# fjarri-attic/pyfft

Measured on AMD Instinct MI355X. Metric: batched_c2c_fft_gflops_5NlogN_1d_n2^20, higher is better.
Workload: dtype f32

## Files before the change

### include/mifft.h

```cpp
#ifndef MIFFT_H
#define MIFFT_H

#include <stddef.h>
#include <stdint.h>

#ifdef __cplusplus
extern "C" {
#endif

#define MIFFT_ABI_VERSION 6

#define MIFFT_E_INVALID      (-1)
#define MIFFT_E_UNSUPPORTED  (-2)
#define MIFFT_E_NODEVICE     (-3)

#define MIFFT_F32 0
#define MIFFT_F64 1

#define MIFFT_INTERLEAVED 0
#define MIFFT_SPLIT       1

#define MIFFT_FLAG_SRC_INTERLEAVED 1
#define MIFFT_FLAG_DST_INTERLEAVED 2
#define MIFFT_FLAG_STREAM_SRC 4
// ... 28 lines not shown
    int32_t src;
    int32_t dst;
    int32_t flags;
} mifft_pass;

typedef struct mifft_device_props {
    char    name[256];
    char    gcn_arch[64];
    int32_t compute_units;
    int32_t wavefront_size;
    int32_t max_threads_per_block;
    int32_t max_grid_x;
    int64_t lds_bytes_per_block;
    int64_t total_mem_bytes;
    int32_t clock_khz;
    int32_t l2_bytes;
    int64_t llc_bytes;
    int32_t num_xcc;
    int32_t reserved0;
} mifft_device_props;

int         mifft_abi_version(void);
const char *mifft_last_error(void);
#define MIFFT_DEBUG_NO_ND2 0
#define MIFFT_DEBUG_NO_WAVE 2
#define MIFFT_DEBUG_FORCE_WAVE 3
#define MIFFT_DEBUG_ALT_ROWS 5
#define MIFFT_DEBUG_PAIR 6
#define MIFFT_DEBUG_STORE 7
#define MIFFT_DEBUG_ROWS_ND 8
#define MIFFT_DEBUG_NARROW_TILES 9
#define MIFFT_DEBUG_NO_ROWFIRST 10
#define MIFFT_DEBUG_PAIR_LANES 12
#define MIFFT_DEBUG_KEYS 13
int mifft_debug_set(int32_t key, int32_t value);
int mifft_debug_set_default(int32_t key, int32_t value);
int mifft_debug_get(int32_t key);
int mifft_debug_last_pair_lanes_form(void);

int mifft_device_count(int *count);
int mifft_set_device(int device);
int mifft_get_device(int *device);
int mifft_device_props_get(int device, mifft_device_props *props);
int mifft_malloc(void **ptr, size_t nbytes);
int mifft_free(void *ptr);
int mifft_memset(void *ptr, int value, size_t nbytes, mifft_stream_t stream);
int mifft_memcpy_h2d(void *dst, const void *src, size_t nbytes, mifft_stream_t stream);
int mifft_memcpy_d2h(void *dst, const void *src, size_t nbytes, mifft_stream_t stream);
int mifft_memcpy_d2d(void *dst, const void *src, size_t nbytes, mifft_stream_t stream);
int mifft_host_alloc(void **ptr, size_t nbytes);
int mifft_host_free(void *ptr);
int mifft_memcpy_d2h_async(void *dst, const void *src, size_t nbytes, mifft_stream_t stream);
int mifft_stream_create(mifft_stream_t *stream);
int mifft_stream_destroy(mifft_stream_t stream);
int mifft_stream_sync(mifft_stream_t stream);
int mifft_device_sync(void);
typedef void *mifft_graph_t;
int mifft_stream_is_capturing(mifft_stream_t stream, int32_t *capturing);
int mifft_stream_begin_capture(mifft_stream_t stream);
int mifft_stream_end_capture(mifft_stream_t stream, mifft_graph_t *graph);
int mifft_graph_launch(mifft_graph_t graph, mifft_stream_t stream);
int mifft_graph_destroy(mifft_graph_t graph);
int mifft_event_create(mifft_event_t *event);
int mifft_event_destroy(mifft_event_t event);
int mifft_event_record(mifft_event_t event, mifft_stream_t stream);
int mifft_event_sync(mifft_event_t event);
int mifft_event_query(mifft_event_t event);
int mifft_stream_wait_event(mifft_stream_t stream, mifft_event_t event);
int mifft_event_elapsed_ms(float *ms, mifft_event_t start, mifft_event_t stop);


// ... 163 lines not shown
```

### pyfft_amd/_debug.py

```python
import os


def forced_strategy():
    return os.environ.get("PYFFT_AMD_STRATEGY", "auto")


def pipeline_chunk_bytes(default):
    return (int(os.environ.get("PYFFT_AMD_PIPE_MB", "0")) << 20) or default


def no_nd_generic():
    return bool(os.environ.get("PYFFT_AMD_NO_ND_GENERIC"))


def pipeline_streams(default):
    return int(os.environ.get("PYFFT_AMD_PIPE_STREAMS", "0")) or default


def slab_bytes(default):
    return (int(os.environ.get("PYFFT_AMD_SLAB_MB", "0")) << 20) or default


def no_slabs():
    return bool(os.environ.get("PYFFT_AMD_NO_SLABS"))
# ... 42 lines not shown
    return bool(os.environ.get("PYFFT_AMD_NO_FUSEDP_ALT"))


def no_tiled_kernel():
    return bool(os.environ.get("PYFFT_AMD_NO_TILED"))


def no_mixed_nd():
    return bool(os.environ.get("PYFFT_AMD_NO_MIXED_ND"))


def fused3_lag_ring(lag, ring):
    v = os.environ.get("PYFFT_AMD_FUSED3")
    if v:
        lag, ring = (int(t) for t in v.split(","))
    return lag, ring


def apply_native_switches(native):
    for env, key in (("MIFFT_NO_ND2", native.DEBUG_NO_ND2), ("MIFFT_NO_WAVE", native.DEBUG_NO_WAVE),
                     ("MIFFT_FORCE_WAVE", native.DEBUG_FORCE_WAVE)):
        if os.environ.get(env):
            native.lib.mifft_debug_set_default(key, 1)
    if os.environ.get("MIFFT_STORE"):
        native.lib.mifft_debug_set_default(native.DEBUG_STORE, int(os.environ["MIFFT_STORE"]))
    if os.environ.get("MIFFT_ROWS_ND"):
        native.lib.mifft_debug_set_default(native.DEBUG_ROWS_ND, int(os.environ["MIFFT_ROWS_ND"]))
    if os.environ.get("MIFFT_NARROW_TILES"):
        native.lib.mifft_debug_set_default(native.DEBUG_NARROW_TILES, int(os.environ["MIFFT_NARROW_TILES"]))
    if os.environ.get("MIFFT_PAIR"):
        native.lib.mifft_debug_set_default(native.DEBUG_PAIR, int(os.environ["MIFFT_PAIR"]))
    if os.environ.get("MIFFT_PAIR_LANES"):
        native.lib.mifft_debug_set_default(native.DEBUG_PAIR_LANES, int(os.environ["MIFFT_PAIR_LANES"]))
    if os.environ.get("PYFFT_AMD_NO_SPLIT_ROWFIRST"):
        native.lib.mifft_debug_set_default(native.DEBUG_NO_ROWFIRST, 1)
```

### pyfft_amd/_native.py

```python

import ctypes
import os

_HERE = os.path.dirname(os.path.abspath(__file__))
LIB_PATH = os.path.join(_HERE, "libmifft.so")

ABI_VERSION = 6
MIFFT_MIXED_MAX_STAGES = 12

E_INVALID = -1
E_UNSUPPORTED = -2
E_NODEVICE = -3

F32, F64 = 0, 1
INTERLEAVED, SPLIT = 0, 1
VARIANT_INTERLEAVED_ONLY = 2
VARIANT_SPLIT_ONLY = 3
VARIANT_OUT_OF_PLACE_ONLY = 4
VARIANT_OUT_OF_PLACE_ANY_SIZE = 5
VARIANT_SPLIT_OUT_OF_PLACE = 6
VARIANT_SPLIT_OUT_OF_PLACE_ANY_SIZE = 7
PASS_COL, PASS_ROW, PASS_ND = 0, 1, 2
FLAG_SRC_INTERLEAVED, FLAG_DST_INTERLEAVED = 1, 2
FLAG_STREAM_SRC, FLAG_STREAM_DST = 4, 8
FLAG_WRITE_THROUGH = 32
FLAG_PAIR_WITH_NEXT = 16
HALF_KERNEL_TILE, HALF_KERNEL_ROW, HALF_KERNEL_ND2, HALF_KERNEL_ND = 1, 2, 3, 4
ND_KERNEL_WAVE, ND_KERNEL_ND2Z, ND_KERNEL_ND2, ND_KERNEL_ND2ZP, ND_KERNEL_ND2P, ND_KERNEL_ND2T, ND_KERNEL_ND = 1, 2, 3, 4, 5, 6, 7
FUSED2_COUNTER_STRIDE = 64


def fused2_counter_bytes(outer):
    return FUSED2_COUNTER_STRIDE * 4 * (9 + 2 * int(outer))


DEBUG_NO_ND2, DEBUG_NO_WAVE, DEBUG_FORCE_WAVE, DEBUG_ALT_ROWS, DEBUG_PAIR, DEBUG_STORE = 0, 2, 3, 5, 6, 7
DEBUG_ROWS_ND = 8
DEBUG_NARROW_TILES = 9
DEBUG_NO_ROWFIRST = 10
DEBUG_PAIR_LANES = 12
DEBUG_KEYS = 13


class MifftPass(ctypes.Structure):
    _fields_ = [
        ("kind", ctypes.c_int32),
        ("precision", ctypes.c_int32),
        ("layout", ctypes.c_int32),
        ("inverse", ctypes.c_int32),
        ("L", ctypes.c_int32),
        ("variant", ctypes.c_int32),
        ("M", ctypes.c_int64),
        ("S", ctypes.c_int64),
        ("outer", ctypes.c_int64),
        ("outer_stride_in", ctypes.c_int64),
        ("outer_stride_out", ctypes.c_int64),
        ("scale", ctypes.c_double),
        ("tw_L", ctypes.c_void_p),
        ("tw_lo", ctypes.c_void_p),
        ("tw_hi", ctypes.c_void_p),
        ("tw_shift", ctypes.c_int32),
        ("src", ctypes.c_int32),
        ("dst", ctypes.c_int32),
        ("flags", ctypes.c_int32),
    ]


class MifftCopy(ctypes.Structure):
    _fields_ = [
        ("precision", ctypes.c_int32),
        ("ndim", ctypes.c_int32),
        ("dims", ctypes.c_int64 * 6),
        ("src_stride", ctypes.c_int64 * 6),
        ("dst_stride", ctypes.c_int64 * 6),
# ... 63 lines not shown
class MifftRealPost(ctypes.Structure):
    _fields_ = [
        ("precision", ctypes.c_int32),
        ("inverse", ctypes.c_int32),
        ("nx", ctypes.c_int32),
        ("ny", ctypes.c_int32),
        ("nz", ctypes.c_int32),
        ("reserved", ctypes.c_int32),
        ("outer", ctypes.c_int64),
        ("stride_in", ctypes.c_int64),
        ("stride_out", ctypes.c_int64),
        ("in_", ctypes.c_void_p),
        ("out", ctypes.c_void_p),
        ("tw", ctypes.c_void_p),
        ("scale", ctypes.c_double),
    ]


_vp = ctypes.c_void_p
_vpp = ctypes.POINTER(ctypes.c_void_p)
_i32 = ctypes.c_int32
_sz = ctypes.c_size_t
_pass_p = ctypes.POINTER(MifftPass)
_sync_p = ctypes.POINTER(MifftFusedSync)
_buf3 = ctypes.c_void_p * 3

PROTOTYPES = {
    "mifft_abi_version": (ctypes.c_int, []),
    "mifft_last_error": (ctypes.c_char_p, []),
    "mifft_debug_set": (ctypes.c_int, [_i32, _i32]),
    "mifft_debug_set_default": (ctypes.c_int, [_i32, _i32]),
    "mifft_debug_get": (ctypes.c_int, [_i32]),
    "mifft_debug_last_pair_lanes_form": (ctypes.c_int, []),
    "mifft_device_count": (ctypes.c_int, [ctypes.POINTER(ctypes.c_int)]),
    "mifft_set_device": (ctypes.c_int, [ctypes.c_int]),
    "mifft_get_device": (ctypes.c_int, [ctypes.POINTER(ctypes.c_int)]),
    "mifft_device_props_get": (ctypes.c_int, [ctypes.c_int, ctypes.POINTER(MifftDeviceProps)]),
    "mifft_malloc": (ctypes.c_int, [_vpp, _sz]),
    "mifft_free": (ctypes.c_int, [_vp]),
    "mifft_memset": (ctypes.c_int, [_vp, ctypes.c_int, _sz, _vp]),
    "mifft_memcpy_h2d": (ctypes.c_int, [_vp, _vp, _sz, _vp]),
    "mifft_memcpy_d2h": (ctypes.c_int, [_vp, _vp, _sz, _vp]),
    "mifft_memcpy_d2d": (ctypes.c_int, [_vp, _vp, _sz, _vp]),
    "mifft_host_alloc": (ctypes.c_int, [_vpp, _sz]),
    "mifft_host_free": (ctypes.c_int, [_vp]),
    "mifft_memcpy_d2h_async": (ctypes.c_int, [_vp, _vp, _sz, _vp]),
    "mifft_stream_create": (ctypes.c_int, [_vpp]),
    "mifft_stream_destroy": (ctypes.c_int, [_vp]),
    "mifft_stream_sync": (ctypes.c_int, [_vp]),
    "mifft_device_sync": (ctypes.c_int, []),
    "mifft_stream_is_capturing": (ctypes.c_int, [_vp, ctypes.POINTER(ctypes.c_int32)]),
    "mifft_stream_begin_capture": (ctypes.c_int, [_vp]),
    "mifft_stream_end_capture": (ctypes.c_int, [_vp, _vpp]),
    "mifft_graph_launch": (ctypes.c_int, [_vp, _vp]),
    "mifft_graph_destroy": (ctypes.c_int, [_vp]),
    "mifft_event_create": (ctypes.c_int, [_vpp]),
    "mifft_event_destroy": (ctypes.c_int, [_vp]),
    "mifft_event_record": (ctypes.c_int, [_vp, _vp]),
    "mifft_event_sync": (ctypes.c_int, [_vp]),
    "mifft_event_query": (ctypes.c_int, [_vp]),
    "mifft_stream_wait_event": (ctypes.c_int, [_vp, _vp]),
    "mifft_event_elapsed_ms": (ctypes.c_int, [ctypes.POINTER(ctypes.c_float), _vp, _vp]),
    "mifft_nd_max_points_for": (ctypes.c_int, [_i32]),
    "mifft_nd_shape_supported": (ctypes.c_int, [_i32, _i32, _i32, _i32, _i32]),
    "mifft_pass_supported": (ctypes.c_int, [_i32, _i32, _i32, _i32]),
    "mifft_launch_pass": (ctypes.c_int, [_pass_p, _vp, _vp, _vp, _vp, _vp]),
# ... 94 lines not shown
```

### pyfft_amd/csrc/fft_col2.hpp

```cpp
#pragma once
#include "fft_tile.hpp"

namespace mifft {

template <int A, int E, typename T> __device__ __forceinline__ cplx<T> mul_w16A(cplx<T> v) {
    if constexpr (A == 4)
        return mul_w64<E, T>(v);
    else
        return mul_w32<E, T>(v);
}

template <typename T> struct ColStageTw {
    cplx<T> s1, s2, s3, s4, s5, s6, s7, s8;
    __device__ __forceinline__ void init(const cplx<T>* twL, int i0, int step = 1) {
        load(twL, i0, step);
        finish();
    }
    __device__ __forceinline__ void load(const cplx<T>* twL, int i0, int step = 1) {
        s1 = twL[step * i0]; s2 = twL[2 * step * i0]; s4 = twL[4 * step * i0]; s8 = twL[8 * step * i0];
    }
    __device__ __forceinline__ void finish() {
        s3 = cmul<T>(s1, s2); s5 = cmul<T>(s4, s1); s6 = cmul<T>(s4, s2); s7 = cmul<T>(s4, s3);
    }
    template <int k> __device__ __forceinline__ cplx<T> get() const {
        if constexpr (k == 1) return s1;
        else if constexpr (k == 2) return s2;
        else if constexpr (k == 3) return s3;
        else if constexpr (k == 4) return s4;
        else if constexpr (k == 5) return s5;
        else if constexpr (k == 6) return s6;
        else if constexpr (k == 7) return s7;
        else if constexpr (k == 8) return s8;
        else if constexpr (k == 9) return cmul<T>(s8, s1);
        else if constexpr (k == 10) return cmul<T>(s8, s2);
        else if constexpr (k == 11) return cmul<T>(s8, s3);
        else if constexpr (k == 12) return cmul<T>(s8, s4);
        else if constexpr (k == 13) return cmul<T>(s8, s5);
        else if constexpr (k == 14) return cmul<T>(s8, s6);
        else return cmul<T>(s8, s7);
    }
};

template <int A, bool TR, int ESZ = 8> struct Col2Lds {
    static constexpr int PITCH = TR ? 17 : 16;
    static constexpr int BUF = 16 * 16 * PITCH;
    static constexpr bool DOUBLE = A > 2 && ESZ <= 8;
    static constexpr bool HALF = ESZ > 8;
    static constexpr int ELEMS = HALF ? (BUF + 1) / 2 : (DOUBLE ? 2 : 1) * BUF;
};

struct TileNoHook {
    __device__ __forceinline__ void operator()() const {}
};

__device__ __forceinline__ void pair_swap(cplx<float>& lo, cplx<float>& hi) {
    const float lx = lo.x, ly = lo.y, hx = hi.x, hy = hi.y;
    const auto rx = __builtin_amdgcn_permlane32_swap(__builtin_bit_cast(unsigned, lx), __builtin_bit_cast(unsigned, hx), false, false);
    const auto ry = __builtin_amdgcn_permlane32_swap(__builtin_bit_cast(unsigned, ly), __builtin_bit_cast(unsigned, hy), false, false);
    const unsigned ax = rx[0], bx = rx[1], ay = ry[0], by = ry[1];
    lo.x = __builtin_bit_cast(float, ax); hi.x = __builtin_bit_cast(float, bx);
    lo.y = __builtin_bit_cast(float, ay); hi.y = __builtin_bit_cast(float, by);
}

template <typename T, int A, bool TR, bool TW, bool SPLIT, bool WT = false, bool NTIN = false, bool NTOUT = false,
          bool SPLIT_OUT = SPLIT, bool WIDE = false, bool PAIR_IN = false, bool PAIR_OUT = false, typename LdsPtr = cplx<T>*,
          typename Hook = TileNoHook>
__device__ __forceinline__ void col2_tile(const TileArgs& a, const long long o_in, const long long o_out,
                                          const long long rem0, LdsPtr lds, Hook hook = Hook(), const int tid_in = -1) {
    constexpr int L = A * 256;
    constexpr int PPT = A * 16;
    constexpr int PITCH = Col2Lds<A, TR, sizeof(cplx<T>)>::PITCH;
    constexpr int BUF = Col2Lds<A, TR, sizeof(cplx<T>)>::BUF;
    constexpr bool kDoubleBuf = Col2Lds<A, TR, sizeof(cplx<T>)>::DOUBLE;
    constexpr bool kHalf = Col2Lds<A, TR, sizeof(cplx<T>)>::HALF;
    static_assert(!(PAIR_IN || PAIR_OUT) || (sizeof(T) == 4 && !WIDE && !kHalf), "paired lanes: fp32 16-column tiles only");
    static_assert(!PAIR_IN || !SPLIT, "PAIR_IN: interleaved input only");
    static_assert(!PAIR_OUT || !SPLIT_OUT, "PAIR_OUT: interleaved output only");
    typedef T vec4 __attribute__((ext_vector_type(4)));

    int tid = tid_in >= 0 ? tid_in : (int)threadIdx.x;
    asm volatile("" : "+v"(tid));
    const int upper = (tid >> 5) & 1;
    const int pair_i = ((tid & 7) << 1) | upper, pair_j = ((tid >> 6) << 2) | ((tid >> 3) & 3);
    const int cg = PAIR_IN ? pair_i : WIDE ? (tid & 31) : (tid & 15), b0 = PAIR_IN ? pair_j : WIDE ? (tid >> 5) : (tid >> 4);
    const int c = cg & 15;
    if constexpr (WIDE) lds = lds + (cg >> 4) * Col2Lds<A, TR, sizeof(cplx<T>)>::ELEMS;
    int logMS = a.logMS, logS = a.logS;
    asm volatile("" : "+s"(logMS), "+s"(logS));
    const cplx<T>* twL = reinterpret_cast<const cplx<T>*>(a.tw_L);
    const T csign = a.inverse ? (T)-1 : (T)1;

    cplx<T> v[PPT];
    {
        const long long ubase = o_in * a.ostride_in + rem0;
        const unsigned voff = (((unsigned)b0 << logMS) + (unsigned)cg);
        if constexpr (PAIR_IN) {
            const char* src = reinterpret_cast<const char*>(reinterpret_cast<const cplx<T>*>(a.in0) + ubase);
            const unsigned vb = ((((unsigned)b0 + (upper ? 16u * A : 0u)) << logMS) + (unsigned)(cg & ~1)) * (unsigned)sizeof(cplx<T>);
            static_for<PPT / 2>([&](auto mm) {
                constexpr int k = 2 * mm, ia = k >> 4, b1 = k & 15;
                const char* p = src + (((long long)(b1 * 16 * A + ia * 16) << logMS) * (long long)sizeof(cplx<T>));
                vec4 w;
                if constexpr (NTIN)
                    w = __builtin_nontemporal_load(reinterpret_cast<const vec4*>(p + vb));
                else
                    w = *reinterpret_cast<const vec4*>(p + vb);
                v[k].x = w.x; v[k].y = w.y; v[k + 1].x = w.z; v[k + 1].y = w.w;
            });
        } else if constexpr (!SPLIT) {
            const char* src = reinterpret_cast<const char*>(reinterpret_cast<const cplx<T>*>(a.in0) + ubase);
            const unsigned vb = voff * (unsigned)sizeof(cplx<T>);
            static_for<PPT>([&](auto kk) {
                constexpr int k = kk, ia = k >> 4, b1 = k & 15;
                const char* p = src + (((long long)(b1 * 16 * A + ia * 16) << logMS) * (long long)sizeof(cplx<T>));
                if constexpr (NTIN)
                    v[k] = __builtin_nontemporal_load(reinterpret_cast<const cplx<T>*>(p + vb));
                else
                    v[k] = *reinterpret_cast<const cplx<T>*>(p + vb);
            });
        } else {
            const char* sre = reinterpret_cast<const char*>(reinterpret_cast<const T*>(a.in0) + ubase);
            const char* sim = reinterpret_cast<const char*>(reinterpret_cast<const T*>(a.in1) + ubase);
            const unsigned vb = voff * (unsigned)sizeof(T);
            static_for<PPT>([&](auto kk) {
                constexpr int k = kk, ia = k >> 4, b1 = k & 15;
                const long long off = ((long long)(b1 * 16 * A + ia * 16) << logMS) * (long long)sizeof(T);
                if constexpr (NTIN) {
                    v[k].x = __builtin_nontemporal_load(reinterpret_cast<const T*>(sre + off + vb));
                    v[k].y = __builtin_nontemporal_load(reinterpret_cast<const T*>(sim + off + vb));
                } else {
                    v[k].x = *reinterpret_cast<const T*>(sre + off + vb);
                    v[k].y = *reinterpret_cast<const T*>(sim + off + vb);
                }
            });
// ... 56 lines not shown
                constexpr int ia = aa;
                t[ia] = v[ia * 16 + qb1];
            });
            Dft<A, T>::run(t);
            v[qb1] = t[0];
            static_for<A - 1>([&](auto qq) {
                constexpr int qa = qq + 1;
                v[qa * 16 + qb1] = cmul<T>(t[qa], twA[qq]);
            });
        });
    }
    __builtin_amdgcn_sched_barrier(0);
    hook();

    const int u = PAIR_OUT ? (TR ? pair_i : pair_j) : TR ? c : b0;
    const int c2 = PAIR_OUT ? (TR ? pair_j : pair_i) : TR ? b0 : c;
    const int c2g = WIDE ? ((cg & 16) + c2) : c2;
    const int c2s = (PAIR_OUT && !TR) ? (c2g & ~1) : c2g;
    const int us = (PAIR_OUT && TR) ? (u & ~1) : u;
    const long long l0 = rem0 >> logS;
    const long long jp0 = rem0 & ((1ll << logS) - 1);
    const unsigned dl = (unsigned)(((rem0 + c2s) >> logS) - l0);
    const unsigned djp = (unsigned)(((rem0 + c2s) & ((1ll << logS) - 1)) - jp0);
    const unsigned l = PAIR_OUT ? (unsigned)((rem0 + c2g) >> logS) : (unsigned)l0 + dl;
    const T sx = (T)a.scale;
    const T sy = a.inverse ? -sx : sx;
    cplx<T> sxy;
    sxy.x = sx;
    sxy.y = sy;
    const cplx<T>* twlo = reinterpret_cast<const cplx<T>*>(a.tw_lo);
    const cplx<T>* twhi = reinterpret_cast<const cplx<T>*>(a.tw_hi);
    const int tw_shift = a.tw_shift;
    const unsigned lomask = (1u << tw_shift) - 1u;
    const long long oubase = TR ? (a.ostride_out * o_out + rem0 * L) : (a.ostride_out * o_out + ((l0 * L) << logS) + jp0);
    const unsigned ovoff = (TR ? ((unsigned)c2g * L + (unsigned)us) : ((((unsigned)dl * L + (unsigned)us) << logS) + djp)) +
                           ((PAIR_OUT && upper) ? (TR ? 16u * A : ((16u * A) << logS)) : 0u);

    cplx<T> nlo[TW ? 4 : 1], nhi[TW ? 4 : 1], sstep_lo, sstep_hi;
    auto look_ahead = [&](auto qq) {
        constexpr int qa = qq;
        if constexpr (TW) {
            static_for<4>([&](auto jj) {
                constexpr int j = jj;
                const unsigned e = l * (unsigned)(qa * 16 + u + 64 * A * j);
                nlo[j] = twlo[e & lomask];
                nhi[j] = twhi[e >> tw_shift];
            });
        }
    };
    if constexpr (TW) {
        const unsigned e = l * (16u * A);
        sstep_lo = twlo[e & lomask];
        sstep_hi = twhi[e >> tw_shift];
        look_ahead(IC<0>{});
        __builtin_amdgcn_sched_barrier(0);
    }

    static_for<A>([&](auto rr) {
        constexpr int qa = rr;
        LdsPtr buf = lds + (kDoubleBuf ? (qa & 1) * BUF : 0);
        if constexpr (!kDoubleBuf && qa > 0) __syncthreads();
        cplx<T> x[16];
        if constexpr (!kHalf) {
            static_for<16>([&](auto ss) {
                constexpr int qb1 = ss;
                if constexpr (TR)
                    buf[(b0 * 16 + c) * PITCH + qb1] = v[qa * 16 + qb1];
                else
                    buf[(b0 * 16 + qb1) * 16 + c] = v[qa * 16 + qb1];
// ... 27 lines not shown
                        w = sb[(bi * 16 + c2) * PITCH + u];
                    else
                        w = sb[(bi * 16 + u) * 16 + c2];
                    if constexpr (comp == 0) x[bi].x = w; else x[bi].y = w;
                });
            });
        }
        cplx<T> anchor[TW ? 4 : 1];
        cplx<T> sstep;
        if constexpr (TW) {
            static_for<4>([&](auto jj) { anchor[jj] = cmul<T>(nlo[jj], nhi[jj]); });
            sstep = cmul<T>(sstep_lo, sstep_hi);
            __builtin_amdgcn_sched_barrier(0);
            if constexpr (qa + 1 < A) {
                look_ahead(IC<qa + 1>{});
                __builtin_amdgcn_sched_barrier(0);
            }
        }
        Dft<16, T>::run(x);
        if constexpr (TW) {
            static_for<4>([&](auto jj) {
                constexpr int j = jj;
                cplx<T> cur = anchor[j];
                static_for<4>([&](auto ii) {
                    constexpr int qb0 = 4 * j + ii;
                    x[qb0] = cmul<T>(x[qb0], cur);
                    if constexpr (ii < 3) cur = cmul<T>(cur, sstep);
                });
            });
        }
        if constexpr (PAIR_OUT) {
            static_for<8>([&](auto hh) {
                constexpr int qb0 = 2 * hh;
                const long long gu = TR ? (oubase + qb0 * 16 * A + 16 * qa)
                                        : (oubase + ((long long)(qb0 * 16 * A + 16 * qa) << logS));
                cplx<T> r0 = x[qb0] * sxy, r1 = x[qb0 + 1] * sxy;
                pair_swap(r0, r1);
                vec4 w;
                w.x = r0.x; w.y = r0.y; w.z = r1.x; w.w = r1.y;
                char* p = reinterpret_cast<char*>(reinterpret_cast<cplx<T>*>(a.out0) + gu);
                if constexpr (WT)
                    store_b128_sc1(p, ovoff * (unsigned)sizeof(cplx<T>), __builtin_bit_cast(unsigned __attribute__((ext_vector_type(4))), w));
                else if constexpr (NTOUT)
                    __builtin_nontemporal_store(w, reinterpret_cast<vec4*>(p + ovoff * (unsigned)sizeof(cplx<T>)));
                else
                    *reinterpret_cast<vec4*>(p + ovoff * (unsigned)sizeof(cplx<T>)) = w;
            });
        } else {
        static_for<16>([&](auto qq) {
            constexpr int qb0 = qq;
            const long long gu = TR ? (oubase + qb0 * 16 * A + 16 * qa)
                                    : (oubase + ((long long)(qb0 * 16 * A + 16 * qa) << logS));
            const cplx<T> r = x[qb0] * sxy;
            if constexpr (!SPLIT_OUT) {
                char* p = reinterpret_cast<char*>(reinterpret_cast<cplx<T>*>(a.out0) + gu);
                if constexpr (WT) {
                    if constexpr (sizeof(cplx<T>) == 8)
                        __hip_atomic_store(reinterpret_cast<unsigned long long*>(p + ovoff * (unsigned)sizeof(cplx<T>)),
                                           __builtin_bit_cast(unsigned long long, r), __ATOMIC_RELAXED, __HIP_MEMORY_SCOPE_AGENT);
                    else
                        store_wt<T>(p, ovoff * (unsigned)sizeof(cplx<T>), r);
                } else if constexpr (NTOUT) {
                    __builtin_nontemporal_store(r, reinterpret_cast<cplx<T>*>(p + ovoff * (unsigned)sizeof(cplx<T>)));
                } else {
                    *reinterpret_cast<cplx<T>*>(p + ovoff * (unsigned)sizeof(cplx<T>)) = r;
                }
            } else {
                char* pr = reinterpret_cast<char*>(reinterpret_cast<T*>(a.out0) + gu);
// ... 53 lines not shown
```

### pyfft_amd/csrc/fft_fused2.hpp

```cpp
#pragma once
#include "fft_col2.hpp"
#include "fft_col2w.hpp"
#include "fft_col3.hpp"

namespace mifft {

constexpr unsigned kFusedCS = 64u;

struct FusedCtl {
    unsigned* counters;
    unsigned* counters_next;
    unsigned* err;
    unsigned lines;
    unsigned batch;
    unsigned lag;
    unsigned ring;
    unsigned tiles0;
    unsigned tiles1;
};

struct FusedArgs {
    TileArgs p0;
    TileArgs p1;
    FusedCtl c;
// ... 146 lines not shown
        if (it.pass == 2u) {
            fused_flush(pend);
            continue;
        }
        if (it.pass == 0u) {
            if (it.dep != nullptr) fused_wait_ge<false>(it.dep, it.target, seen, err, pend);
            else fused_flush(pend);
            if constexpr (EARLY) tile0(it.t, it.slot, it.tile, hook);
            else tile0(it.t, it.slot, it.tile, TileNoHook());
            pend.ctr = wdone + kFusedCS * it.t;
        } else {
            fused_wait_ge<true>(it.dep, it.target, seen, err, pend);
            if constexpr (EARLY) tile1(it.slot, it.t, it.tile, hook);
            else tile1(it.slot, it.t, it.tile, TileNoHook());
            fused_signal_read(rdone + kFusedCS * it.t);
        }
    }
    fused_flush(pend);
}

template <unsigned PER0, unsigned PER1, bool EARLY, typename TILE0, typename TILE1>
__device__ __forceinline__ void fused_loop(const FusedCtl& f, unsigned* s_item, TILE0&& tile0, TILE1&& tile1) {
    if (f.counters_next != nullptr) {
        for (unsigned i = blockIdx.x * blockDim.x + threadIdx.x; i < f.lines; i += gridDim.x * blockDim.x) {
            f.counters_next[i * kFusedCS] = 0u;
            f.counters_next[i * kFusedCS + 1u] = 0u;
        }
    }
    FusedPending pend = {};
    fused_list<PER0, PER1, EARLY>(f, s_item, tile0, tile1, pend);
}

constexpr int kPairIn = 1, kPairOut = 2;
template <typename T, int A0, int A1, bool SPLIT, int NT, int PAIR0 = 0, int PAIR1 = 0>
__global__ void __launch_bounds__(256, 2) fft_fused2_kernel(const FusedArgs f) {
    static_assert((PAIR0 | PAIR1) == 0 || (sizeof(T) == 4 && A0 == 4 && A1 == 4 && !SPLIT && NT == 1), "paired lanes: <float, 4, 4, false, 1> only");
    constexpr int E0 = Col2Lds<A0, true, sizeof(cplx<T>)>::ELEMS, E1 = Col2Lds<A1, false, sizeof(cplx<T>)>::ELEMS;
    __shared__ __attribute__((aligned(16))) cplx<T> lds[E0 > E1 ? E0 : E1];
    __shared__ unsigned s_item;
    constexpr unsigned per0 = A0 > A1 ? 1u : (unsigned)(A1 / A0);
    constexpr unsigned per1 = A1 > A0 ? 1u : (unsigned)(A0 / A1);
    fused_loop<per0, per1, !SPLIT && sizeof(T) == 4>(
        f.c, &s_item,
        [&](unsigned t, unsigned slot, unsigned tile, auto hook) {
            col2_tile<T, A0, true, true, SPLIT, true, NT != 0, false, false, false, (PAIR0 & kPairIn) != 0, (PAIR0 & kPairOut) != 0>(
                f.p0, (long long)t, (long long)slot, (long long)tile * 16, lds, hook);
        },
        [&](unsigned slot, unsigned t, unsigned tile, auto hook) {
            col2_tile<T, A1, false, false, false, NT == 2, false, NT == 1, SPLIT, false, (PAIR1 & kPairIn) != 0, (PAIR1 & kPairOut) != 0>(
                f.p1, (long long)slot, (long long)t, (long long)tile * 16, lds, hook);
        });
}

template <int A0, int A1, bool TWOD, bool NT = false, bool SPLIT = true>
__global__ void __launch_bounds__(512, 2) fft_fused2s_kernel(const FusedArgs f) {
    constexpr int E0 = Col2Lds<A0, true, sizeof(cplx<float>)>::ELEMS, E1 = Col2Lds<A1, TWOD, sizeof(cplx<float>)>::ELEMS;
    constexpr int E = E0 > E1 ? E0 : E1;
    __shared__ __attribute__((aligned(16))) cplx<float> lds[2 * E];
    __shared__ unsigned s_item;
    constexpr unsigned per0 = A0 > A1 ? 1u : (unsigned)(A1 / A0);
    constexpr unsigned per1 = A1 > A0 ? 1u : (unsigned)(A0 / A1);
    fused_loop<per0, per1, false>(
        f.c, &s_item,
        [&](unsigned t, unsigned slot, unsigned item, auto hook) {
            int tid = threadIdx.x;
            asm volatile("" : "+v"(tid));
            col2_tile<float, A0, true, !TWOD, SPLIT, true, NT, false, false, true>(f.p0, (long long)t, (long long)slot, (long long)item * 32, lds, hook, tid);
        },
        [&](unsigned slot, unsigned t, unsigned item, auto hook) {
            int tid = threadIdx.x;
            asm volatile("" : "+v"(tid));
            col2_tile<float, A1, TWOD, false, false, false, false, NT, SPLIT, true>(f.p1, (long long)slot, (long long)t, (long long)item * 32, lds, hook, tid);
        });
}

template <int A0, int A1>
__global__ void __launch_bounds__(256, 2) fft_fused2w_kernel(const FusedArgs f) {
    constexpr int E0 = Col2wLds<true>::ELEMS, E1 = Col2wLds<false>::ELEMS;
    __shared__ __attribute__((aligned(16))) cplx<float> lds[E0 > E1 ? E0 : E1];
    __shared__ unsigned s_item;
    constexpr unsigned per0 = A0 > A1 ? 1u : (unsigned)(A1 / A0);
    constexpr unsigned per1 = A1 > A0 ? 1u : (unsigned)(A0 / A1);
// ... 97 lines not shown
```

### pyfft_amd/csrc/fft_fused2_f32.hip

```cpp
#include "../../include/mifft.h"
#include "mifft_internal.h"
#include "fft_fused2.hpp"

namespace {
constexpr int kPairLanesDefault = 3;
int launch_1024(const mifft::FusedArgs* f, unsigned grid, hipStream_t s) {
    constexpr int kPairAll = mifft::kPairIn | mifft::kPairOut;
    const int sw = mifft_debug_get(MIFFT_DEBUG_PAIR_LANES);
    int form = sw == 0 ? kPairLanesDefault : sw - 1;
    if (form != 0 && form != 3) return -2;
    if ((((uintptr_t)f->p0.in0 | (uintptr_t)f->p1.out0) & 15) != 0) form = 0;
    if (form == 3) hipLaunchKernelGGL((mifft::fft_fused2_kernel<float, 4, 4, false, 1, kPairAll, kPairAll>), dim3(grid), dim3(256), 0, s, *f);
    else hipLaunchKernelGGL((mifft::fft_fused2_kernel<float, 4, 4, false, 1>), dim3(grid), dim3(256), 0, s, *f);
    mifft_note_pair_lanes_form(form);
    return (int)hipGetLastError();
}

template <int A0, int A1> int launch(const mifft::FusedArgs* f, int split, unsigned grid, hipStream_t s) {
    if constexpr (A0 < A1) {
        return -2;
    } else {
        const int store = mifft_debug_get(MIFFT_DEBUG_STORE);
        if (mifft_debug_get(MIFFT_DEBUG_NARROW_TILES) == 1 || store == 2 || store == 3) return -2;
        if (split) {
            hipLaunchKernelGGL((mifft::fft_fused2s_kernel<A0, A1, false, true>), dim3(grid), dim3(512), 0, s, *f);
        } else if constexpr (A0 == 4 && A1 == 4) {
            return launch_1024(f, grid, s);
        } else if constexpr (A0 == 4) {
            hipLaunchKernelGGL((mifft::fft_fused2_kernel<float, A0, A1, false, 1>), dim3(grid), dim3(256), 0, s, *f);
        } else {
            return -2;
        }
        return (int)hipGetLastError();
    }
}
}

extern "C" int mifft_fused2_f32_launch(int L0, int L1, const mifft::FusedArgs* f, int split, unsigned grid, hipStream_t s) {
    if (L0 == 2048 && L1 == 2048) {
        if (split) hipLaunchKernelGGL((mifft::fft_fused3_kernel<float, 4, 4, true, true>), dim3(grid), dim3(512), 0, s, *f);
        else hipLaunchKernelGGL((mifft::fft_fused3_kernel<float, 4, 4, false, true>), dim3(grid), dim3(512), 0, s, *f);
        return (int)hipGetLastError();
    }
    if (L0 == 2048 && L1 == 1024) {
        if (split) hipLaunchKernelGGL((mifft::fft_fused3_kernel<float, 4, 2, true, true>), dim3(grid), dim3(512), 0, s, *f);
        else hipLaunchKernelGGL((mifft::fft_fused3_kernel<float, 4, 2, false, true>), dim3(grid), dim3(512), 0, s, *f);
        return (int)hipGetLastError();
// ... 27 lines not shown
```

### pyfft_amd/csrc/mifft_internal.h

```cpp
#pragma once
#include <hip/hip_runtime.h>
#include "../../include/mifft.h"
#include "fft_tile.hpp"
#include "fft_fused2.hpp"
#include "fft_nd.hpp"
#include "fft_wave.hpp"
#include "fft_pair.hpp"
#include "fft_nd2t.hpp"
#include "fft_fusedp.hpp"

extern "C" {
int mifft_dispatch_col_f32(int L, int tr, int variant, const mifft::TileArgs* a, hipStream_t s, int query_only);
int mifft_dispatch_row_f32(int L, int variant, const mifft::TileArgs* a, hipStream_t s, int query_only);
int mifft_dispatch_col_f64(int L, int tr, int variant, const mifft::TileArgs* a, hipStream_t s, int query_only);
int mifft_dispatch_row_f64(int L, int variant, const mifft::TileArgs* a, hipStream_t s, int query_only);
int mifft_nd_max_points(int f64);
int mifft_nd_launch(int f64, long long n, const mifft::NdArgs* a, hipStream_t s);
int mifft_nd2_f32_supported(int x, int y, int z);
int mifft_nd2_f32_launch(int x, int y, int z, const mifft::TileArgs* a, hipStream_t s);
int mifft_nd2_f64_supported(int x, int y, int z);
int mifft_nd2_f64_launch(int x, int y, int z, const mifft::TileArgs* a, hipStream_t s);
int mifft_fused2_f32_launch(int L0, int L1, const mifft::FusedArgs* f, int split, unsigned grid, hipStream_t s);
void mifft_note_pair_lanes_form(int form);
int mifft_fused2dw_f32(int ny, int nx, const mifft::FusedArgs* f, unsigned grid, hipStream_t s, int query, unsigned* tiles0, unsigned* tiles1);
int mifft_fused2r_f32(int ny, int nx, const mifft::FusedArgs* f, unsigned grid, hipStream_t s, int query);
int mifft_fused2w_f32_launch(int L0, int L1, const mifft::FusedArgs* f, unsigned grid, hipStream_t s);
int mifft_fused2d_f32_launch(int ny, int nx, const mifft::FusedArgs* f, int split, unsigned grid, hipStream_t s);
int mifft_fused3d_f64_launch(int ny, int nx, const mifft::FusedArgs* f, int split, unsigned grid, hipStream_t s);
int mifft_fusedx_f64(int L0, int L1, const mifft::FusedArgs* f, unsigned grid, hipStream_t s, int query, unsigned* tiles0, unsigned* tiles1);
int mifft_fused3_f64_launch(int L0, int L1, const mifft::FusedArgs* f, int split, unsigned grid, hipStream_t s);
int mifft_aux_copy_launch(const struct mifft_copy* c, const void* s0, const void* s1, void* d0, void* d1, hipStream_t s);
int mifft_aux_mul_rows_launch(int f64, void* a, const void* b, long long rows, long long n, hipStream_t s);
int mifft_aux_mul_spectrum_launch(int f64, void* data, const void* spectrum, long long items, long long points, long long spectrum_pitch,
                                  int correlate, double scale, hipStream_t s);
int mifft_aux_mismatch_launch(const void* a, const void* b, unsigned long long words, unsigned long long* count, hipStream_t s);
int mifft_aux_zero_launch(void* p, unsigned long long nbytes, hipStream_t s);
int mifft_wave_supported(int f64, int N);
int mifft_wave_launch(int f64, int N, const mifft::WaveArgs* a, int max_blocks, hipStream_t s);
int mifft_wave_16x16_launch(const mifft::WaveArgs* a, int max_blocks, hipStream_t s);
int mifft_pair_f64(int kind, int k0, int k1, int k2, int split, const mifft::PairArgs* a, hipStream_t s, int query, int* width);
int mifft_pair_f32(int kind, int k0, int k1, int k2, int split, const mifft::PairArgs* a, hipStream_t s, int query, int* width);
int mifft_fusedp(int f64, int split, int x, int y, int z, const mifft::FusedPairArgs* f, unsigned grid, hipStream_t s, int query, int* r0,
                 unsigned* tiles0, unsigned* tiles1);
int mifft_fusedp_more(int f64, int split, int x, int y, int z, const mifft::FusedPairArgs* f, unsigned grid, hipStream_t s, int query, int* r0,
                      unsigned* tiles0, unsigned* tiles1);
int mifft_nd2t(int f64, int x, int y, int z, const mifft::TileArgs* a, const mifft::TiledGeom* g, hipStream_t s, int query);
int mifft_nd2t_split_in(int f64, int x, int y, int z, const mifft::TileArgs* a, const mifft::TiledGeom* g, hipStream_t s, int query);
int mifft_nd2t_split(int f64, int x, int y, int z, const mifft::TileArgs* a, const mifft::TiledGeom* g, hipStream_t s, int query);
int mifft_nd2p(int f64, int x, int y, int z, const mifft::TileArgs* a, hipStream_t s, int query);
int mifft_nd2zp(int f64, int x, int y, int z, const mifft::TileArgs* a, hipStream_t s, int query);
int mifft_mixed_supported_impl(int f64, int n);
int mifft_mixed_radices_impl(int n, int32_t* radix);
int mifft_mixed_launch(int f64, int n, long long rows, long long stride_in, long long stride_out, long long inner, const void* in,
                       void* out, const void* tw, int flags, double scale, hipStream_t s);
int mifft_mixed_long_split_impl(int f64, long long n, int* n1, int* n2);
int mifft_mixed_long_launch(int f64, int n1, int n2, long long batch, const void* in, void* mid, void* out, const void* tw1, const void* tw2,
// ... 52 lines not shown
```

### pyfft_amd/csrc/mifft_runtime.cpp

```cpp
#include <hip/hip_runtime.h>
#include <hsa/hsa.h>
#include <hsa/hsa_ext_amd.h>

#include <atomic>
#include <cstdarg>
#include <cstdio>
#include <cstring>
#include <cstdlib>
#include <initializer_list>

#include "../../include/mifft.h"
#include "mifft_internal.h"
#include "fft_conv_row.hpp"

namespace {

thread_local char g_err[512] = "";
std::atomic<int> g_debug_default[MIFFT_DEBUG_KEYS];
thread_local int t_debug_value[MIFFT_DEBUG_KEYS];
thread_local unsigned t_debug_mask = 0;
thread_local int t_pair_lanes_form = -1;
struct DebugSwitches {
    int operator[](int key) const {
        return ((t_debug_mask >> key) & 1u) ? t_debug_value[key] : g_debug_default[key].load(std::memory_order_relaxed);
    }
};
const DebugSwitches g_debug;

int set_err(int code, const char* fmt, ...) {
    va_list ap;
    va_start(ap, fmt);
    vsnprintf(g_err, sizeof(g_err), fmt, ap);
    va_end(ap);
    return code;
}

int hip_check(hipError_t e, const char* what) {
    if (e == hipSuccess) return 0;
    return set_err((int)e, "%s: %s (%d)", what, hipGetErrorString(e), (int)e);
}

int launched(int rc) {
    if (rc == -1) return set_err(MIFFT_E_INVALID, "grid too large");
    return hip_check((hipError_t)rc, "kernel launch");
}

bool is_pow2(long long v) { return v > 0 && (v & (v - 1)) == 0; }
bool bad_precision(int precision) { return precision != MIFFT_F32 && precision != MIFFT_F64; }
long long complex_bytes(int precision) { return precision == MIFFT_F64 ? 16 : 8; }
bool misaligned(uintptr_t mask, std::initializer_list<const void*> ptrs) {
    uintptr_t all = 0;
    for (const void* p : ptrs) all |= (uintptr_t)p;
    return (all & mask) != 0;
}
// ... 382 lines not shown
    c->tiles1 = tiles1;
    if (!sync->counters_next) {
        hipStreamCaptureStatus st = hipStreamCaptureStatusNone;
        if (hipStreamIsCapturing(stream, &st) == hipSuccess && st == hipStreamCaptureStatusActive) {
            const int rz = mifft_aux_zero_launch(sync->counters, MIFFT_FUSED2_COUNTER_BYTES(outer), stream);
            return hip_check((hipError_t)rz, "kernel launch");
        }
        return hip_check(hipMemsetAsync(sync->counters, 0, MIFFT_FUSED2_COUNTER_BYTES(outer), stream), "hipMemsetAsync");
    }
    return 0;
}

template <typename F> F* row_dispatcher(int32_t precision, F* f32, F* f64) { return precision == MIFFT_F64 ? f64 : f32; }

}

extern "C" {

int mifft_abi_version(void) { return MIFFT_ABI_VERSION; }
int mifft_debug_set(int32_t key, int32_t value) {
    if (!debug_key_ok(key)) return set_err(MIFFT_E_INVALID, "bad debug key %d", key);
    t_debug_value[key] = value;
    t_debug_mask |= 1u << key;
    return 0;
}
int mifft_debug_set_default(int32_t key, int32_t value) {
    if (!debug_key_ok(key)) return set_err(MIFFT_E_INVALID, "bad debug key %d", key);
    g_debug_default[key].store(value, std::memory_order_relaxed);
    return 0;
}
int mifft_debug_get(int32_t key) { return (key >= 0 && key < MIFFT_DEBUG_KEYS) ? g_debug[key] : 0; }
void mifft_note_pair_lanes_form(int form) { t_pair_lanes_form = form; }
int mifft_debug_last_pair_lanes_form(void) { return t_pair_lanes_form; }
const char* mifft_last_error(void) { return g_err; }

int mifft_device_count(int* count) {
    if (!count) return set_err(MIFFT_E_INVALID, "null argument");
    hipError_t e = hipGetDeviceCount(count);
    if (e == hipErrorNoDevice) {
        *count = 0;
        (void)hipGetLastError();
        return 0;
    }
    return hip_check(e, "hipGetDeviceCount");
}
int mifft_set_device(int device) { return hip_check(hipSetDevice(device), "hipSetDevice"); }
int mifft_get_device(int* device) { return hip_check(hipGetDevice(device), "hipGetDevice"); }

int mifft_device_props_get(int device, mifft_device_props* props) {
    if (!props) return set_err(MIFFT_E_INVALID, "null argument");
    hipDeviceProp_t p;
    int rc = hip_check(hipGetDeviceProperties(&p, device), "hipGetDeviceProperties");
    if (rc) return rc;
    memset(props, 0, sizeof(*props));
    snprintf(props->name, sizeof(props->name), "%s", p.name);
    snprintf(props->gcn_arch, sizeof(props->gcn_arch), "%s", p.gcnArchName);
    props->compute_units = p.multiProcessorCount;
    props->wavefront_size = p.warpSize;
    props->max_threads_per_block = p.maxThreadsPerBlock;
    props->max_grid_x = p.maxGridSize[0];
    props->lds_bytes_per_block = (int64_t)p.sharedMemPerBlock;
    props->total_mem_bytes = (int64_t)p.totalGlobalMem;
    props->clock_khz = p.clockRate;
    props->l2_bytes = p.l2CacheSize;
    probe_memory_system(p, &props->llc_bytes, &props->num_xcc);
    return 0;
// ... 961 lines not shown
```

Baseline: 22600.

## Add bit-permuted ring layout for fused 1024x1024 intermediate buffer

Adds a compile-time bit-permutation layout for the intermediate ring buffer between the two stages of the fused persistent 1024x1024 fp32 kernel. The intermediate is stored as [i][j][n2%16][k1%16], so each 16x16 tile written by stage one and read by stage two is contiguous rather than strided by 1024. The goal is better write/read locality, fewer DRAM pages and fewer cache lines touched per tile. The layout is on by default for the paired-lane form, with a debug switch to fall back, and it adds index arithmetic plus a risk of addressing mistakes in the permuted offsets.

```diff
diff --git a/include/mifft.h b/include/mifft.h
--- a/include/mifft.h
+++ b/include/mifft.h
@@ -84,11 +84,13 @@
 #define MIFFT_DEBUG_NARROW_TILES 9
 #define MIFFT_DEBUG_NO_ROWFIRST 10
 #define MIFFT_DEBUG_PAIR_LANES 12
-#define MIFFT_DEBUG_KEYS 13
+#define MIFFT_DEBUG_RING_LAYOUT 13
+#define MIFFT_DEBUG_KEYS 14
 int mifft_debug_set(int32_t key, int32_t value);
 int mifft_debug_set_default(int32_t key, int32_t value);
 int mifft_debug_get(int32_t key);
 int mifft_debug_last_pair_lanes_form(void);
+int mifft_debug_last_ring_layout(void);
 
 int mifft_device_count(int *count);
 int mifft_set_device(int device);
diff --git a/pyfft_amd/_debug.py b/pyfft_amd/_debug.py
--- a/pyfft_amd/_debug.py
+++ b/pyfft_amd/_debug.py
@@ -98,5 +98,7 @@
         native.lib.mifft_debug_set_default(native.DEBUG_PAIR, int(os.environ["MIFFT_PAIR"]))
     if os.environ.get("MIFFT_PAIR_LANES"):
         native.lib.mifft_debug_set_default(native.DEBUG_PAIR_LANES, int(os.environ["MIFFT_PAIR_LANES"]))
+    if os.environ.get("MIFFT_RING_LAYOUT"):
+        native.lib.mifft_debug_set_default(native.DEBUG_RING_LAYOUT, int(os.environ["MIFFT_RING_LAYOUT"]))
     if os.environ.get("PYFFT_AMD_NO_SPLIT_ROWFIRST"):
         native.lib.mifft_debug_set_default(native.DEBUG_NO_ROWFIRST, 1)
diff --git a/pyfft_amd/_native.py b/pyfft_amd/_native.py
--- a/pyfft_amd/_native.py
+++ b/pyfft_amd/_native.py
@@ -39,7 +39,8 @@
 DEBUG_NARROW_TILES = 9
 DEBUG_NO_ROWFIRST = 10
 DEBUG_PAIR_LANES = 12
-DEBUG_KEYS = 13
+DEBUG_RING_LAYOUT = 13
+DEBUG_KEYS = 14
 
 
 class MifftPass(ctypes.Structure):
@@ -169,6 +170,7 @@
     "mifft_debug_set_default": (ctypes.c_int, [_i32, _i32]),
     "mifft_debug_get": (ctypes.c_int, [_i32]),
     "mifft_debug_last_pair_lanes_form": (ctypes.c_int, []),
+    "mifft_debug_last_ring_layout": (ctypes.c_int, []),
     "mifft_device_count": (ctypes.c_int, [ctypes.POINTER(ctypes.c_int)]),
     "mifft_set_device": (ctypes.c_int, [ctypes.c_int]),
     "mifft_get_device": (ctypes.c_int, [ctypes.POINTER(ctypes.c_int)]),
diff --git a/pyfft_amd/csrc/fft_col2.hpp b/pyfft_amd/csrc/fft_col2.hpp
--- a/pyfft_amd/csrc/fft_col2.hpp
+++ b/pyfft_amd/csrc/fft_col2.hpp
@@ -1,5 +1,6 @@
 #pragma once
 #include "fft_tile.hpp"
+#include "fft_ring_layout.hpp"
 
 namespace mifft {
 
@@ -63,8 +64,8 @@
 }
 
 template <typename T, int A, bool TR, bool TW, bool SPLIT, bool WT = false, bool NTIN = false, bool NTOUT = false,
-          bool SPLIT_OUT = SPLIT, bool WIDE = false, bool PAIR_IN = false, bool PAIR_OUT = false, typename LdsPtr = cplx<T>*,
-          typename Hook = TileNoHook>
+          bool SPLIT_OUT = SPLIT, bool WIDE = false, bool PAIR_IN = false, bool PAIR_OUT = false, int RING = 0,
+          typename LdsPtr = cplx<T>*, typename Hook = TileNoHook>
 __device__ __forceinline__ void col2_tile(const TileArgs& a, const long long o_in, const long long o_out,
                                           const long long rem0, LdsPtr lds, Hook hook = Hook(), const int tid_in = -1) {
     constexpr int L = A * 256;
@@ -76,6 +77,10 @@
     static_assert(!(PAIR_IN || PAIR_OUT) || (sizeof(T) == 4 && !WIDE && !kHalf), "paired lanes: fp32 16-column tiles only");
     static_assert(!PAIR_IN || !SPLIT, "PAIR_IN: interleaved input only");
     static_assert(!PAIR_OUT || !SPLIT_OUT, "PAIR_OUT: interleaved output only");
+    constexpr bool kRingOut = RING != 0 && TR, kRingIn = RING != 0 && !TR;
+    static_assert(RING >= 0 && RING < kRingLayouts, "no such ring layout");
+    static_assert(RING == 0 || (sizeof(T) == 4 && A == 4 && !SPLIT && !SPLIT_OUT && PAIR_IN && PAIR_OUT && (TR ? (TW && WT) : (!TW && !WT))),
+                  "ring layouts: the paired-lane fp32 1024 x 1024 persistent kernel only");
     typedef T vec4 __attribute__((ext_vector_type(4)));
 
     int tid = tid_in >= 0 ? tid_in : (int)threadIdx.x;
@@ -95,11 +100,14 @@
         const long long ubase = o_in * a.ostride_in + rem0;
         const unsigned voff = (((unsigned)b0 << logMS) + (unsigned)cg);
         if constexpr (PAIR_IN) {
-            const char* src = reinterpret_cast<const char*>(reinterpret_cast<const cplx<T>*>(a.in0) + ubase);
-            const unsigned vb = ((((unsigned)b0 + (upper ? 16u * A : 0u)) << logMS) + (unsigned)(cg & ~1)) * (unsigned)sizeof(cplx<T>);
+            const char* src = reinterpret_cast<const char*>(reinterpret_cast<const cplx<T>*>(a.in0) +
+                                                            (kRingIn ? o_in * a.ostride_in + (long long)ring_offset<RING>(0u, (unsigned)rem0) : ubase));
+            const unsigned vb = (kRingIn ? ring_offset<RING>(((unsigned)b0 & 15u) + (upper ? 16u * A : 0u), (unsigned)(cg & 14))
+                                         : ((((unsigned)b0 + (upper ? 16u * A : 0u)) << logMS) + (unsigned)(cg & ~1))) * (unsigned)sizeof(cplx<T>);
             static_for<PPT / 2>([&](auto mm) {
                 constexpr int k = 2 * mm, ia = k >> 4, b1 = k & 15;
-                const char* p = src + (((long long)(b1 * 16 * A + ia * 16) << logMS) * (long long)sizeof(cplx<T>));
+                const char* p = src + (kRingIn ? (long long)ring_offset<RING>(b1 * 16 * A + ia * 16, 0u) * (long long)sizeof(cplx<T>)
+                                               : (((long long)(b1 * 16 * A + ia * 16) << logMS) * (long long)sizeof(cplx<T>)));
                 vec4 w;
                 if constexpr (NTIN)
                     w = __builtin_nontemporal_load(reinterpret_cast<const vec4*>(p + vb));
@@ -222,9 +230,12 @@
     const cplx<T>* twhi = reinterpret_cast<const cplx<T>*>(a.tw_hi);
     const int tw_shift = a.tw_shift;
     const unsigned lomask = (1u << tw_shift) - 1u;
-    const long long oubase = TR ? (a.ostride_out * o_out + rem0 * L) : (a.ostride_out * o_out + ((l0 * L) << logS) + jp0);
-    const unsigned ovoff = (TR ? ((unsigned)c2g * L + (unsigned)us) : ((((unsigned)dl * L + (unsigned)us) << logS) + djp)) +
-                           ((PAIR_OUT && upper) ? (TR ? 16u * A : ((16u * A) << logS)) : 0u);
+    const long long oubase = kRingOut ? (a.ostride_out * o_out + (long long)ring_offset<RING>((unsigned)rem0, 0u))
+                             : TR     ? (a.ostride_out * o_out + rem0 * L)
+                                      : (a.ostride_out * o_out + ((l0 * L) << logS) + jp0);
+    const unsigned ovoff = kRingOut ? ring_offset<RING>((unsigned)c2g & 15u, ((unsigned)us & 14u) + (upper ? 16u * A : 0u))
+                                    : (TR ? ((unsigned)c2g * L + (unsigned)us) : ((((unsigned)dl * L + (unsigned)us) << logS) + djp)) +
+                                          ((PAIR_OUT && upper) ? (TR ? 16u * A : ((16u * A) << logS)) : 0u);
 
     cplx<T> nlo[TW ? 4 : 1], nhi[TW ? 4 : 1], sstep_lo, sstep_hi;
     auto look_ahead = [&](auto qq) {
@@ -318,8 +329,9 @@
         if constexpr (PAIR_OUT) {
             static_for<8>([&](auto hh) {
                 constexpr int qb0 = 2 * hh;
-                const long long gu = TR ? (oubase + qb0 * 16 * A + 16 * qa)
-                                        : (oubase + ((long long)(qb0 * 16 * A + 16 * qa) << logS));
+                const long long gu = kRingOut ? (oubase + (long long)ring_offset<RING>(0u, qb0 * 16 * A + 16 * qa))
+                                     : TR     ? (oubase + qb0 * 16 * A + 16 * qa)
+                                              : (oubase + ((long long)(qb0 * 16 * A + 16 * qa) << logS));
                 cplx<T> r0 = x[qb0] * sxy, r1 = x[qb0 + 1] * sxy;
                 pair_swap(r0, r1);
                 vec4 w;
diff --git a/pyfft_amd/csrc/fft_fused2.hpp b/pyfft_amd/csrc/fft_fused2.hpp
--- a/pyfft_amd/csrc/fft_fused2.hpp
+++ b/pyfft_amd/csrc/fft_fused2.hpp
@@ -202,9 +202,10 @@
 }
 
 constexpr int kPairIn = 1, kPairOut = 2;
-template <typename T, int A0, int A1, bool SPLIT, int NT, int PAIR0 = 0, int PAIR1 = 0>
+template <typename T, int A0, int A1, bool SPLIT, int NT, int PAIR0 = 0, int PAIR1 = 0, int RING = 0>
 __global__ void __launch_bounds__(256, 2) fft_fused2_kernel(const FusedArgs f) {
     static_assert((PAIR0 | PAIR1) == 0 || (sizeof(T) == 4 && A0 == 4 && A1 == 4 && !SPLIT && NT == 1), "paired lanes: <float, 4, 4, false, 1> only");
+    static_assert(RING == 0 || (PAIR0 == (kPairIn | kPairOut) && PAIR1 == (kPairIn | kPairOut)), "ring layouts: <float, 4, 4, false, 1> with every stream paired only");
     constexpr int E0 = Col2Lds<A0, true, sizeof(cplx<T>)>::ELEMS, E1 = Col2Lds<A1, false, sizeof(cplx<T>)>::ELEMS;
     __shared__ __attribute__((aligned(16))) cplx<T> lds[E0 > E1 ? E0 : E1];
     __shared__ unsigned s_item;
@@ -213,11 +214,11 @@
     fused_loop<per0, per1, !SPLIT && sizeof(T) == 4>(
         f.c, &s_item,
         [&](unsigned t, unsigned slot, unsigned tile, auto hook) {
-            col2_tile<T, A0, true, true, SPLIT, true, NT != 0, false, false, false, (PAIR0 & kPairIn) != 0, (PAIR0 & kPairOut) != 0>(
+            col2_tile<T, A0, true, true, SPLIT, true, NT != 0, false, false, false, (PAIR0 & kPairIn) != 0, (PAIR0 & kPairOut) != 0, RING>(
                 f.p0, (long long)t, (long long)slot, (long long)tile * 16, lds, hook);
         },
         [&](unsigned slot, unsigned t, unsigned tile, auto hook) {
-            col2_tile<T, A1, false, false, false, NT == 2, false, NT == 1, SPLIT, false, (PAIR1 & kPairIn) != 0, (PAIR1 & kPairOut) != 0>(
+            col2_tile<T, A1, false, false, false, NT == 2, false, NT == 1, SPLIT, false, (PAIR1 & kPairIn) != 0, (PAIR1 & kPairOut) != 0, RING>(
                 f.p1, (long long)slot, (long long)t, (long long)tile * 16, lds, hook);
         });
 }
diff --git a/pyfft_amd/csrc/fft_fused2_f32.hip b/pyfft_amd/csrc/fft_fused2_f32.hip
--- a/pyfft_amd/csrc/fft_fused2_f32.hip
+++ b/pyfft_amd/csrc/fft_fused2_f32.hip
@@ -4,15 +4,21 @@
 
 namespace {
 constexpr int kPairLanesDefault = 3;
+constexpr int kRingLayoutDefault = 1;
 int launch_1024(const mifft::FusedArgs* f, unsigned grid, hipStream_t s) {
     constexpr int kPairAll = mifft::kPairIn | mifft::kPairOut;
-    const int sw = mifft_debug_get(MIFFT_DEBUG_PAIR_LANES);
+    const int sw = mifft_debug_get(MIFFT_DEBUG_PAIR_LANES), rsw = mifft_debug_get(MIFFT_DEBUG_RING_LAYOUT);
     int form = sw == 0 ? kPairLanesDefault : sw - 1;
     if (form != 0 && form != 3) return -2;
     if ((((uintptr_t)f->p0.in0 | (uintptr_t)f->p1.out0) & 15) != 0) form = 0;
-    if (form == 3) hipLaunchKernelGGL((mifft::fft_fused2_kernel<float, 4, 4, false, 1, kPairAll, kPairAll>), dim3(grid), dim3(256), 0, s, *f);
-    else hipLaunchKernelGGL((mifft::fft_fused2_kernel<float, 4, 4, false, 1>), dim3(grid), dim3(256), 0, s, *f);
+    if (rsw < 0 || rsw > mifft::kRingLayouts) return -2;
+    if (form == 0 && rsw > 1) return -2;
+    const int layout = form == 0 ? 0 : rsw == 0 ? kRingLayoutDefault : rsw - 1;
+    if (form == 0) hipLaunchKernelGGL((mifft::fft_fused2_kernel<float, 4, 4, false, 1>), dim3(grid), dim3(256), 0, s, *f);
+    else if (layout == 0) hipLaunchKernelGGL((mifft::fft_fused2_kernel<float, 4, 4, false, 1, kPairAll, kPairAll>), dim3(grid), dim3(256), 0, s, *f);
+    else hipLaunchKernelGGL((mifft::fft_fused2_kernel<float, 4, 4, false, 1, kPairAll, kPairAll, 1>), dim3(grid), dim3(256), 0, s, *f);
     mifft_note_pair_lanes_form(form);
+    mifft_note_ring_layout(layout);
     return (int)hipGetLastError();
 }
 
diff --git a/pyfft_amd/csrc/fft_ring_layout.hpp b/pyfft_amd/csrc/fft_ring_layout.hpp
--- /dev/null
+++ b/pyfft_amd/csrc/fft_ring_layout.hpp
@@ -0,0 +1,52 @@
+#pragma once
+
+namespace mifft {
+
+constexpr int kRingLogK1 = 10;
+constexpr int kRingBits = 20;
+constexpr int kRingLayouts = 2;
+
+struct RingField {
+    int from, width, to;
+};
+
+template <int LAYOUT> struct RingLayout;
+template <> struct RingLayout<0> {
+    static constexpr int N = 1;
+    static constexpr RingField f[N] = {{0, 20, 0}};
+};
+template <> struct RingLayout<1> {
+    static constexpr int N = 4;
+    static constexpr RingField f[N] = {{0, 4, 0}, {10, 4, 4}, {4, 6, 8}, {14, 6, 14}};
+};
+
+template <int N> constexpr bool ring_is_permutation(const RingField (&f)[N]) {
+    unsigned from = 0u, to = 0u;
+    for (int i = 0; i < N; ++i) {
+        if (f[i].width <= 0 || f[i].from < 0 || f[i].to < 0 || f[i].from + f[i].width > kRingBits || f[i].to + f[i].width > kRingBits)
+            return false;
+        const unsigned m = (1u << f[i].width) - 1u;
+        if ((from & (m << f[i].from)) != 0u || (to & (m << f[i].to)) != 0u) return false;
+        from |= m << f[i].from;
+        to |= m << f[i].to;
+    }
+    return from == (1u << kRingBits) - 1u && to == (1u << kRingBits) - 1u;
+}
+static_assert(ring_is_permutation(RingLayout<0>::f) && ring_is_permutation(RingLayout<1>::f),
+              "a ring layout must be a permutation of bits 0 ... 19 of the slot offset");
+
+template <int LAYOUT, int I = 0> __host__ __device__ constexpr unsigned ring_offset(unsigned x) {
+    if constexpr (I == RingLayout<LAYOUT>::N) {
+        return 0u;
+    } else {
+        constexpr RingField fl = RingLayout<LAYOUT>::f[I];
+        return (((x >> fl.from) & ((1u << fl.width) - 1u)) << fl.to) | ring_offset<LAYOUT, I + 1>(x);
+    }
+}
+template <int LAYOUT> __host__ __device__ constexpr unsigned ring_offset(unsigned n2, unsigned k1) {
+    return ring_offset<LAYOUT>((n2 << kRingLogK1) | k1);
+}
+static_assert(ring_offset<1>(17u, 35u) == (1u << 14) + (2u << 8) + (1u << 4) + 3u && ring_offset<0>(17u, 35u) == 17u * 1024u + 35u,
+              "ring layout 1: [i][j][n2 % 16][k1 % 16]");
+
+}
diff --git a/pyfft_amd/csrc/mifft_internal.h b/pyfft_amd/csrc/mifft_internal.h
--- a/pyfft_amd/csrc/mifft_internal.h
+++ b/pyfft_amd/csrc/mifft_internal.h
@@ -22,6 +22,7 @@
 int mifft_nd2_f64_launch(int x, int y, int z, const mifft::TileArgs* a, hipStream_t s);
 int mifft_fused2_f32_launch(int L0, int L1, const mifft::FusedArgs* f, int split, unsigned grid, hipStream_t s);
 void mifft_note_pair_lanes_form(int form);
+void mifft_note_ring_layout(int layout);
 int mifft_fused2dw_f32(int ny, int nx, const mifft::FusedArgs* f, unsigned grid, hipStream_t s, int query, unsigned* tiles0, unsigned* tiles1);
 int mifft_fused2r_f32(int ny, int nx, const mifft::FusedArgs* f, unsigned grid, hipStream_t s, int query);
 int mifft_fused2w_f32_launch(int L0, int L1, const mifft::FusedArgs* f, unsigned grid, hipStream_t s);
diff --git a/pyfft_amd/csrc/mifft_runtime.cpp b/pyfft_amd/csrc/mifft_runtime.cpp
--- a/pyfft_amd/csrc/mifft_runtime.cpp
+++ b/pyfft_amd/csrc/mifft_runtime.cpp
@@ -20,6 +20,7 @@
 thread_local int t_debug_value[MIFFT_DEBUG_KEYS];
 thread_local unsigned t_debug_mask = 0;
 thread_local int t_pair_lanes_form = -1;
+thread_local int t_ring_layout = -1;
 struct DebugSwitches {
     int operator[](int key) const {
         return ((t_debug_mask >> key) & 1u) ? t_debug_value[key] : g_debug_default[key].load(std::memory_order_relaxed);
@@ -468,6 +469,8 @@
 int mifft_debug_get(int32_t key) { return (key >= 0 && key < MIFFT_DEBUG_KEYS) ? g_debug[key] : 0; }
 void mifft_note_pair_lanes_form(int form) { t_pair_lanes_form = form; }
 int mifft_debug_last_pair_lanes_form(void) { return t_pair_lanes_form; }
+void mifft_note_ring_layout(int layout) { t_ring_layout = layout; }
+int mifft_debug_last_ring_layout(void) { return t_ring_layout; }
 const char* mifft_last_error(void) { return g_err; }
 
 int mifft_device_count(int* count) {
```

New measurement: 22700, median of 6. About the same (+0.4%).
